# sunyinqi0508/AQuery2

Measured on AMD Instinct MI355X. Metric: rows/sec on h2o groupby 1e9-row, higher is better.
Workload: dtype int64

## Files before the change

### aquery2_amd/capi.py

```python
import ctypes as C
import os
import weakref

import numpy as np

HERE = os.path.dirname(os.path.abspath(__file__))

INT32, FLOAT, STR, DOUBLE, LDOUBLE, INT64, INT128, INT16, DATE, TIME, INT8 = range(11)
UINT32, UINT64, UINT128, UINT16, UINT8, BOOL = 11, 12, 13, 14, 15, 16
TIMESTAMP = 18
ERROR = 22
I128 = np.dtype([("lo", "<u8"), ("hi", "<i8")])
U128 = np.dtype([("lo", "<u8"), ("hi", "<u8")])
TAG2NP = {
    INT8: np.dtype(np.int8), INT16: np.dtype(np.int16), INT32: np.dtype(np.int32), INT64: np.dtype(np.int64),
    UINT8: np.dtype(np.uint8), UINT16: np.dtype(np.uint16), UINT32: np.dtype(np.uint32), UINT64: np.dtype(np.uint64),
    FLOAT: np.dtype(np.float32), DOUBLE: np.dtype(np.float64), BOOL: np.dtype(np.uint8), INT128: I128, UINT128: U128,
}
NP2TAG = {v: k for k, v in TAG2NP.items() if k != BOOL}
NP2TAG[np.dtype(np.bool_)] = BOOL
VEC_VEC, VEC_SCALAR, SCALAR_VEC = 0, 1, 2
LAYOUT_ROW, LAYOUT_FLAT = 0, 1
ORDER_ASC, ORDER_DESC, ORDER_NEG = 0, 1, 2
SEL_LOWER, SEL_UPPER = 0, 1
# ... 52 lines not shown
JOIN_INNER, JOIN_LEFT, JOIN_SEMI, JOIN_ANTI = range(4)
JOIN_ROUTE_PACKED, JOIN_ROUTE_WIDE, JOIN_ROUTE_LDS, JOIN_ROUTE_HBM = 1, 2, 4, 8
JOIN_KEYS_PROTOTYPES = {
    "aqg_join_keys_count": [C.c_void_p, C.c_int, C.c_int, C.c_void_p, C.c_void_p, C.c_uint32, C.c_void_p, C.c_uint32, C.POINTER(C.c_uint64)],
    "aqg_join_keys_pairs": [C.c_void_p, C.c_int, C.c_int, C.c_void_p, C.c_void_p, C.c_uint32, C.c_void_p, C.c_uint32, C.c_void_p, C.c_void_p,
                            C.c_uint64, C.POINTER(C.c_uint64)],
    "aqg_join_keys_lookup": [C.c_void_p, C.c_int, C.c_void_p, C.c_void_p, C.c_uint32, C.c_void_p, C.c_uint32, C.c_void_p],
    "aqg_join_last": [C.c_void_p, C.POINTER(C.c_uint32), C.POINTER(C.c_uint32), C.POINTER(C.c_uint32)],
    "aqg_join_tuple_slots": [C.c_int, C.c_void_p, C.c_void_p, C.c_uint32, C.c_uint32, C.c_void_p],
    "aqg_gather_fill": [C.c_void_p, C.c_int, C.c_void_p, C.c_void_p, C.c_uint32, C.c_void_p, C.c_void_p],
}
ASOF_BACKWARD, ASOF_FORWARD = 0, 1
ASOF_STRICT = 1
ASOF_ROUTE_LDS, ASOF_ROUTE_HBM, ASOF_ROUTE_NOKEYS, ASOF_ROUTE_PRESORTED = 1, 2, 4, 8
ASOF_PROTOTYPES = {
    "aqg_join_asof": [C.c_void_p, C.c_int, C.c_int, C.c_int, C.c_void_p, C.c_void_p, C.c_void_p, C.c_uint32, C.c_void_p, C.c_void_p, C.c_uint32,
                      C.c_int, C.c_void_p],
    "aqg_join_asof_last": [C.c_void_p, C.POINTER(C.c_uint32), C.POINTER(C.c_uint32), C.POINTER(C.c_uint32)],
}
STR_ROUTE_HOST, STR_ROUTE_DEVICE, STR_ROUTE_FALLBACK = 1, 2, 4
STR_PROTOTYPES = {
    "aqg_str_encode_last": [C.c_void_p, C.POINTER(C.c_uint32), C.POINTER(C.c_uint32)],
}
PLAN_FAST_LDS, PLAN_SMALL_LDS, PLAN_BIG_LDS, PLAN_DENSE, PLAN_PART_ONE, PLAN_PART_TWO, PLAN_PART_ROUND1, PLAN_PART_WIDE, PLAN_SORTED_TAIL, PLAN_HBM_TABLE, PLAN_BUILD_PARTITIONED, PLAN_GID_PARTITION, PLAN_PACKED_VALUES, PLAN_RANGE_PARTITIONS, PLAN_ROW_EMIT, PLAN_PACKED_KEYS, PLAN_BUILD_LOOKUP = (1 << i for i in range(17))


class AqgError(RuntimeError):
    def __init__(self, what, code, detail=""):
        super().__init__(f"{what}: status {code} {detail}")
        self.code = code


def lib_path():
    return os.path.join(HERE, "libaqg.so")


_LIB = None


def load_library():
    global _LIB
    if _LIB is None:
        p = lib_path()
        if not os.path.exists(p):
            raise FileNotFoundError(f"{p} not built: run `python -c 'import __graft_entry__ as g; g.build()'` "
                                    "or `make -C aquery2_amd/csrc`")
        lib = C.CDLL(p)
# ... 733 lines not shown

    def grouped_flatten(self, gb, x, keep=False):
        xd = self._dev(x)
        out = self.empty(xd.n, xd.dtype)
        self._chk(self.lib.aqg_grouped_flatten(self.ctx, gb.h, xd.tag, C.c_void_p(xd.ptr), C.c_void_p(out.ptr)), "aqg_grouped_flatten")
        return out if keep else out.to_host()

    def grouped_scan(self, gb, op, x, w=0, flat=False, keep=False, out=None):
        xd = self._dev(x)
        ot = self.lib.aqg_scan_out_dtype(op, xd.tag)
        out = out if out is not None else self.empty(xd.n, TAG2NP[ot])
        fn = self.lib.aqg_grouped_scan_flat if flat else self.lib.aqg_grouped_scan
        self._chk(fn(self.ctx, gb.h, op, xd.tag, C.c_void_p(xd.ptr), C.c_uint32(w), C.c_void_p(out.ptr)), "aqg_grouped_scan")
        return out if keep else out.to_host()

    def grouped_reduce_flat(self, gb, op, xflat):
        xd = self._dev(xflat)
        ot = self.lib.aqg_reduce_out_dtype(op, xd.tag)
        out = self.empty(gb.ngroups, TAG2NP[ot])
        self._chk(self.lib.aqg_grouped_reduce_flat(self.ctx, gb.h, op, xd.tag, C.c_void_p(xd.ptr), C.c_void_p(out.ptr)), "aqg_grouped_reduce_flat")
        self.sync()
        return out.to_host()

    def grouped_corr(self, gb, x, y):
        xd, yd = self._dev(x), self._dev(y)
        out = self.empty(gb.ngroups, np.float64)
        self._chk(self.lib.aqg_grouped_corr(self.ctx, gb.h, xd.tag, C.c_void_p(xd.ptr), yd.tag, C.c_void_p(yd.ptr), C.c_void_p(out.ptr)), "aqg_grouped_corr")
        self.sync()
        return out.to_host()

    def grouped_ewise(self, gb, op, v, s, kind=VEC_SCALAR, layout=LAYOUT_ROW, ot=None, keep=False, out=None):
        vd, sd = self._dev(v), self._dev(s)
        if ot is None:
            ot = self.lib.aqg_ewise_out_dtype(op, *((vd.tag, sd.tag) if kind == VEC_SCALAR else (sd.tag, vd.tag)))
        if ot == ERROR:
            raise AqgError("aqg_ewise_out_dtype", ERROR)
        out = out if out is not None else self.empty(vd.n, TAG2NP[ot])
        self._chk(self.lib.aqg_grouped_ewise(self.ctx, gb.h, layout, op, kind, vd.tag, C.c_void_p(vd.ptr), sd.tag, C.c_void_p(sd.ptr), ot,
                                             C.c_void_p(out.ptr)), "aqg_grouped_ewise")
        return out if keep else out.to_host()

    def join_pairs(self, build, probe):
        bd, pd = self._dev(build), self._dev(probe)
        m = C.c_uint64()
        self._chk(self.lib.aqg_join_count(self.ctx, bd.tag, C.c_void_p(bd.ptr), C.c_uint32(bd.n), C.c_void_p(pd.ptr),
                                          C.c_uint32(pd.n), C.byref(m)), "aqg_join_count")
# ... 87 lines not shown
```

### aquery2_amd/csrc/aqg_internal.hpp

```cpp
#pragma once
#include <hip/hip_runtime.h>

#include <cstdint>
#include <cstdio>
#include <cstring>
#include <string>
#include <unordered_map>
#include <vector>

#include "../../include/aqg.h"

struct aqg_pin { void* dptr; size_t bytes; std::vector<std::pair<void*, size_t>> regs; hipEvent_t ev; };

struct aqg_ctx {
    int device = 0;
    hipStream_t stream = nullptr;
    bool own_stream = false;
    int num_cu = 256;
    std::string err;
    char* ws = nullptr;
    size_t ws_cap = 0, ws_off = 0;
    hipEvent_t ev0 = nullptr, ev1 = nullptr;
    hipEvent_t evk0 = nullptr, evk1 = nullptr;
    hipEvent_t ev_flags = nullptr;
// ... 40 lines not shown
            (void)hipGetLastError();  \
            return AQG_ERR_HIP;                                                                \
        }                                                                                      \
    } while (0)

#define AQG_TRY(expr)                          \
    do {                                       \
        int _rc = (expr);                      \
        if (_rc != AQG_OK) return _rc;         \
    } while (0)

static inline int aqg_fail(aqg_ctx* ctx, int code, const char* msg) {
    if (ctx) ctx->err = msg;
    return code;
}
#define AQG_CHECK_ROWS(ctx, n, what) do { if ((uint64_t)(n) > (uint64_t)AQG_MAX_ROWS) return aqg_fail(ctx, AQG_ERR_ARG, what ": more than AQG_MAX_ROWS rows"); } while (0)
static inline uint32_t aqg_ceil_div(uint32_t n, uint32_t d) { return (uint32_t)(((uint64_t)n + d - 1) / d); }

struct aqg_switch_set {
    uint32_t p1_max, sorted_tail_min;
    int p1_bins;
    uint32_t select_small_max, select_split_min;
    double pw_sigma;
    bool disable_p1, disable_p1_cursors, disable_ranged, disable_pw_defer, disable_build_partition, debug_flags, str_host;
};
const aqg_switch_set& aqg_switches();

int aqg_ws_reset(aqg_ctx* ctx);
static inline void* aqg_pool_take(aqg_ctx* ctx, size_t need, size_t* cap) {
    if (ctx->pool_big && ctx->pool_big_cap >= need && ctx->pool_big_cap <= 2 * need) { void* p = ctx->pool_big; *cap = ctx->pool_big_cap; ctx->pool_big = nullptr; ctx->pool_big_cap = 0; return p; }
    int best = -1;
    const size_t slack = need * 4 > ((size_t)64 << 10) ? need * 4 : ((size_t)64 << 10);
    for (int i = 0; i < (int)ctx->pool.size(); ++i)
        if (ctx->pool[i].second >= need && ctx->pool[i].second <= slack && (best < 0 || ctx->pool[i].second < ctx->pool[best].second)) best = i;
    if (best < 0) return nullptr;
    void* p = ctx->pool[best].first;
    *cap = ctx->pool[best].second;
    ctx->pool_bytes -= *cap;
    ctx->pool[best] = ctx->pool.back();
    ctx->pool.pop_back();
    return p;
}
static inline void aqg_pool_give(aqg_ctx* ctx, void* p, size_t cap) {
    if (!p) return;
    if (ctx && cap && cap <= ((size_t)64 << 20) && ctx->pool.size() < 64 && ctx->pool_bytes + cap <= ((size_t)512 << 20)) { ctx->pool.emplace_back(p, cap); ctx->pool_bytes += cap; return; }
    if (ctx && cap > ((size_t)64 << 20) && cap <= ((size_t)8 << 30) && cap > ctx->pool_big_cap) {
        if (ctx->pool_big) (void)hipFree(ctx->pool_big);
// ... 17 lines not shown
    hipError_t e = hipSuccess;
    void* q = aqg_pool_alloc(ctx, need < 256 ? 256 : need, cap, &e);
    if (!q) { ctx->err = std::string("hipMalloc: ") + hipGetErrorString(e); return AQG_ERR_NOMEM; }
    *p = static_cast<T*>(q);
    return AQG_OK;
}
int aqg_ws_alloc(aqg_ctx* ctx, size_t bytes, void** out);
int aqg_ws_ensure(aqg_ctx* ctx, size_t bytes);
template <class T> static inline int aqg_ws_get(aqg_ctx* ctx, size_t count, T** out) {
    void* p = nullptr;
    int rc = aqg_ws_alloc(ctx, count * sizeof(T), &p);
    *out = static_cast<T*>(p);
    return rc;
}
int aqg_host_stage(aqg_ctx* ctx, size_t bytes, void** out);
int aqg_exclusive_scan_u32(aqg_ctx* ctx, uint32_t* d, uint64_t count, uint32_t* bsum);

struct aqg_groupby;
size_t aqg_postproc_ws_bytes(uint32_t n, uint32_t G, int esz);
int aqg_radix_by_group(aqg_ctx* ctx, aqg_groupby* g, uint32_t* row_ids_dev, const void* x, int esz, void* xout, bool ws_managed);
int aqg_group_offsets(aqg_ctx* ctx, const aqg_groupby* g, uint32_t* offsets_dev, uint32_t* bsum);
int aqg_flat_gid(aqg_ctx* ctx, aqg_groupby* g, const uint32_t** gid);
extern "C" int aqg_grouped_reduce_keyed(aqg_ctx* ctx, aqg_groupby* g, const uint32_t* gid_col, int op, int t, const void* x, void* out_dev);

struct aqg_comm;
int aqg_comm_allgather_internal(aqg_comm* c, const void* send_dev, void* recv_dev, size_t bytes);
aqg_ctx* aqg_comm_ctx(aqg_comm* c);
extern "C" int aqg_scan_minmax_seeded(aqg_ctx* ctx, int op, int t, const void* x, uint32_t n, const void* seed_host, void* out);

extern "C" int aqg_stats_dev(aqg_ctx* ctx, int t, const void* x, uint32_t n, int flags, void* out_dev48);
extern "C" int aqg_corr_sums_dev(aqg_ctx* ctx, int tx, const void* x, int ty, const void* y, uint32_t n, void* out_dev80);
int aqg_comm_scratch(aqg_comm* c, size_t send_bytes, size_t recv_bytes, void** send, void** recv);

constexpr int AQG_RED_SUMSQ = 64;

static inline void aqg_kernel_timer_begin(aqg_ctx* ctx) { if (!ctx->evk_frozen) (void)hipEventRecord(ctx->evk0, ctx->stream); }
static inline void aqg_kernel_timer_end(aqg_ctx* ctx) { if (!ctx->evk_frozen) { (void)hipEventRecord(ctx->evk1, ctx->stream); ctx->evk_valid = true; } }

static inline int aqg_check_launch(aqg_ctx* ctx, const char* what) {
    hipError_t e = hipGetLastError();
    if (e != hipSuccess) {
        ctx->err = std::string(what) + ": " + hipGetErrorString(e);
        return AQG_ERR_HIP;
    }
    return AQG_OK;
}
// ... 48 lines not shown
```

### aquery2_amd/csrc/ctx.hip

```cpp
#include <string_view>

#include <mutex>

#include "aqg_internal.hpp"

extern "C" {

const char* aqg_version(void) { return "aquery2_amd 0.1 (gfx950)"; }

size_t aqg_dtype_size(int dt) {
    switch (dt) {
    case AQG_INT8: case AQG_UINT8: case AQG_BOOL: case AQG_CHAR: return 1;
    case AQG_INT16: case AQG_UINT16: return 2;
    case AQG_INT32: case AQG_UINT32: case AQG_FLOAT: return 4;
    case AQG_INT64: case AQG_UINT64: case AQG_DOUBLE: return 8;
    case AQG_INT128: case AQG_UINT128: return 16;
    default: return 0;
    }
}
int aqg_long_type(int dt) {
    if (!aqg_dtype_size(dt)) return AQG_ERROR;
    if (dt_is_fp(dt)) return AQG_DOUBLE;
    return dt_is_unsigned(dt) ? AQG_UINT128 : AQG_INT128;
}
// ... 339 lines not shown
    AQG_HIP(ctx, hipEventElapsedTime(ms, ctx->ev0, ctx->ev1));
    return AQG_OK;
}

int aqg_last_kernel_ms(aqg_ctx* ctx, float* ms) {
    if (!ctx || !ms) return AQG_ERR_ARG;
    if (!ctx->evk_valid) return aqg_fail(ctx, AQG_ERR_ARG, "aqg_last_kernel_ms: no timed kernel yet");
    AQG_HIP(ctx, hipEventSynchronize(ctx->evk1));
    AQG_HIP(ctx, hipEventElapsedTime(ms, ctx->evk0, ctx->evk1));
    return AQG_OK;
}

}

const aqg_switch_set& aqg_switches() {
    auto num = [](const char* name, int dflt) { return getenv(name) ? atoi(getenv(name)) : dflt; };
    auto set = [](const char* name) { return getenv(name) != nullptr; };
    auto unum = [](const char* name, uint32_t dflt) { return getenv(name) ? (uint32_t)strtoul(getenv(name), nullptr, 10) : dflt; };
    static const aqg_switch_set s{
        .p1_max = (uint32_t)num("AQG_P1_MAX", 1024), .sorted_tail_min = (uint32_t)num("AQG_SORTED_TAIL_MIN", 1 << 24), .p1_bins = num("AQG_P1_BINS", 0),
        .select_small_max = unum("AQG_SELECT_SMALL_MAX", 256), .select_split_min = unum("AQG_SELECT_SPLIT_MIN", 1u << 20),
        .pw_sigma = getenv("AQG_PW_SIGMA") ? atof(getenv("AQG_PW_SIGMA")) : 6.0,
        .disable_p1 = set("AQG_DISABLE_P1"), .disable_p1_cursors = set("AQG_DISABLE_P1_CURSORS"), .disable_ranged = set("AQG_DISABLE_RANGED"),
        .disable_pw_defer = set("AQG_DISABLE_PW_DEFER"), .disable_build_partition = set("AQG_DISABLE_BUILD_PARTITION"),
        .debug_flags = set("AQG_DEBUG_FLAGS"), .str_host = set("AQG_STR_HOST")};
    return s;
}

int aqg_ws_reset(aqg_ctx* ctx) {
    ctx->ws_off = 0;
    return AQG_OK;
}
int aqg_ws_ensure(aqg_ctx* ctx, size_t bytes) {
    if (bytes <= ctx->ws_cap) return AQG_OK;
    AQG_HIP(ctx, hipSetDevice(ctx->device));
    AQG_HIP(ctx, hipStreamSynchronize(ctx->stream));
    size_t cap = ctx->ws_cap ? ctx->ws_cap : (size_t)1 << 20;
    while (cap < bytes) cap *= 2;
    if (bytes > ((size_t)4 << 30)) cap = (bytes + (((size_t)1 << 30) - 1)) & ~(((size_t)1 << 30) - 1);
    if (ctx->ws) { hipFree(ctx->ws); ctx->ws = nullptr; ctx->ws_cap = 0; }
    void* p = nullptr;
    hipError_t e = hipMalloc(&p, cap);
    if (e != hipSuccess) { ctx->err = std::string("workspace hipMalloc: ") + hipGetErrorString(e); (void)hipGetLastError(); return AQG_ERR_NOMEM; }
    ctx->ws = static_cast<char*>(p);
    ctx->ws_cap = cap;
    return AQG_OK;
}
// ... 21 lines not shown
```

### aquery2_amd/csrc/groupby.hip

```cpp
#include "groupby_plan.hpp"

size_t aqg_partition_ws_bytes(uint32_t n, int ksz, const AccSpec& as, uint32_t pbits);
int aqg_partition_aggregate(aqg_ctx* ctx, const KeySpec& ks, const AccSpec& as, uint32_t n, uint32_t pbits, uint32_t lcap, int need_count, GTable out, uint32_t out_cap);

int aqg_make_keyspec(aqg_ctx* ctx, int nkeys, const int* dts, const void* const* keys, uint32_t n, KeySpec* ks) {
    if (nkeys < 1 || nkeys > MAXKEYS) return aqg_fail(ctx, AQG_ERR_ARG, "group-by: 1..8 key columns");
    int bits = 0;
    ks->nkeys = nkeys;
    ks->range_known = 0; ks->range_lo = ks->range_hi = 0;
    for (int j = 0; j < nkeys; ++j) {
        if (!(dt_is_num(dts[j]) || dts[j] == AQG_BOOL)) return aqg_fail(ctx, AQG_ERR_DTYPE, "group-by: key dtype");
        if (dt_is_fp(dts[j])) return aqg_fail(ctx, AQG_ERR_DTYPE, "group-by: internal: floating key column reached the packed-key layer");
        if (!keys[j] && n) return aqg_fail(ctx, AQG_ERR_ARG, "group-by: null key column");
        ks->dt[j] = dts[j]; ks->col[j] = keys[j]; ks->shift[j] = bits;
        bits += 8 * (int)aqg_dtype_size(dts[j]);
    }
    ks->wide = bits > 64;
    if (ks->wide) for (int j = 0; j < nkeys; ++j) ks->shift[j] = 0;
    ks->total_bytes = bits / 8;
    return AQG_OK;
}

int aqg_add_acc(Plan* p, int kind, int dt, const void* col, int square, int part) {
    for (int a = 0; a < p->as.nacc; ++a)
// ... 383 lines not shown
    for (int attempt = 0; attempt < 12; ++attempt) {
        if (cur > n && n) cur = n;
        int rc = run_agg(ctx, ks, plan, n, (uint32_t)cur, for_build, h, gt_out, slot_gid_out, occ_out, dense_out);
        for (int again = 0; again < 3 && rc == AQG_ERR_RANGE_MISS; ++again) rc = run_agg(ctx, ks, plan, n, (uint32_t)cur, for_build, h, gt_out, slot_gid_out, occ_out, dense_out);
        if (rc != AQG_ERR_OVERFLOW) { if (rc == AQG_OK) h->hint_used = (uint32_t)cur; return rc; }
        if (n && cur >= n) return aqg_fail(ctx, AQG_ERR_OVERFLOW, "group-by: table overflow at full capacity");
        const uint64_t next = cur < (1ull << 25) && cur * 16 > (1ull << 25) ? (1ull << 25) : cur * 16;
        cur = plan.sj && cur < 3072 && next > 3072 ? 3072 : next;
    }
    return aqg_fail(ctx, AQG_ERR_OVERFLOW, "group-by: table overflow");
}

extern "C" {

void aqg_groupby_destroy(aqg_groupby* g) {
    if (!g) return;
    aqg_ctx* ctx = g->ctx;
    for (int k = 0; k < MAXKEYS; ++k) aqg_pool_give(ctx, g->keys_out[k], g->cap_keys[k]);
    for (int j = 0; j < MAXAGG; ++j) aqg_pool_give(ctx, g->results[j], g->cap_results[j]);
    aqg_pool_give(ctx, g->first_rows, g->cap_first);
    aqg_pool_give(ctx, g->counts, g->cap_counts);
    aqg_pool_give(ctx, g->reversemap, g->cap_rows * 4);
    if (g->scratch) aqg_groupby_destroy(g->scratch);
    if (g->scratch2) aqg_groupby_destroy(g->scratch2);
    if (g->scratch3) aqg_groupby_destroy(g->scratch3);
    aqg_pool_give(ctx, g->flat_off, g->cap_flat_off);
    aqg_pool_give(ctx, g->flat_heads, g->cap_flat_heads);
    aqg_pool_give(ctx, g->flat_short, g->cap_flat_short);
    aqg_pool_give(ctx, g->flat_gid, g->cap_flat_gid);
    if (g->first_rows64) hipFree(g->first_rows64);
    for (int i = 0; i < 2 * MAXKEYS; ++i) if (g->norm_buf[i]) hipFree(g->norm_buf[i]);
    if (g->xkeys) hipFree(g->xkeys);
    if (g->xvals) hipFree(g->xvals);
    delete g;
}
uint32_t aqg_groupby_ngroups(const aqg_groupby* g) { return g ? g->ngroups : 0; }
uint32_t aqg_groupby_nrows(const aqg_groupby* g) { return g ? g->n : 0; }
const uint32_t* aqg_groupby_reversemap(const aqg_groupby* g) { return g && g->has_reversemap ? g->reversemap : nullptr; }
const uint32_t* aqg_groupby_counts(const aqg_groupby* g) { return g && g->has_counts ? g->counts : nullptr; }
const uint32_t* aqg_groupby_first_rows(const aqg_groupby* g) { return g && !g->sharded ? g->first_rows : nullptr; }
uint32_t aqg_groupby_plan(const aqg_groupby* g) { return g ? g->plan_bits : 0; }
const void* aqg_groupby_agg_result(const aqg_groupby* g, int j) { return g && j >= 0 && j < g->nagg ? g->results[j] : nullptr; }

int aqg_groupby_agg(aqg_ctx* ctx, int nkeys, const int* key_dtypes, const void* const* keys, int naggs, const int* ops,
                    const int* val_dtypes, const void* const* vals, uint32_t n, uint32_t max_groups_hint, aqg_groupby** out) {
    if (!ctx || !out || !key_dtypes || !keys) return aqg_fail(ctx, AQG_ERR_ARG, "aqg_groupby_agg: bad argument");
    AQG_CHECK_ROWS(ctx, n, "aqg_groupby_agg");
// ... 50 lines not shown
```

### aquery2_amd/csrc/groupby_handle.hpp

```cpp
#pragma once
#include <cstddef>
#include <cstdint>

struct aqg_ctx;
constexpr int MAXKEYS = 8, MAXACC = 8, MAXAGG = 8;

struct aqg_groupby {
    aqg_ctx* ctx = nullptr;
    uint32_t n = 0, ngroups = 0;
    int nkeys = 0;
    int key_dt[MAXKEYS] = {0};
    int key_esz[MAXKEYS] = {0};
    bool has_counts = false, has_reversemap = false;
    void* keys_out[MAXKEYS] = {nullptr};
    uint32_t* first_rows = nullptr;
    uint32_t* counts = nullptr;
    uint32_t* reversemap = nullptr;
    void* results[MAXAGG] = {nullptr};
    int nagg = 0;
    int res_dt[MAXAGG] = {0};
    size_t cap_keys[MAXKEYS] = {0}, cap_first = 0, cap_counts = 0, cap_rows = 0, cap_results[MAXAGG] = {0};
    uint32_t hint_used = 0;
    uint32_t plan_bits = 0;
    int64_t* first_rows64 = nullptr;
    size_t cap_first64 = 0;
    bool sharded = false;
    int nuser = 0;
    int user_dt[MAXKEYS] = {0};
    const void* user_col[MAXKEYS] = {nullptr};
    int user_norm[MAXKEYS] = {0};
    void* norm_buf[2 * MAXKEYS] = {nullptr};
    size_t cap_norm[2 * MAXKEYS] = {0};
    bool build_assigned = false;
    bool no_lookup_build = false;
    bool no_sorted_tail = false;
    bool no_pack = false;
    bool no_wide_part = false;
    uint32_t wide_rows = 0;
    uint32_t wide_seed = 0;
    bool dense_exact = false;
    bool range_valid = false; int range_nkeys = 0; uint32_t range_n = 0;
    const void* range_col[MAXKEYS] = {}; int range_dt[MAXKEYS] = {}; long long range_min[MAXKEYS] = {}, range_max[MAXKEYS] = {};
    aqg_groupby* scratch = nullptr;
    aqg_groupby* scratch2 = nullptr;
    aqg_groupby* scratch3 = nullptr;
    uint32_t* flat_off = nullptr; uint32_t* flat_heads = nullptr; uint32_t* flat_short = nullptr; uint32_t* flat_gid = nullptr;
    size_t cap_flat_off = 0, cap_flat_heads = 0, cap_flat_short = 0, cap_flat_gid = 0;
    bool flat_valid = false, flat_gid_valid = false;
    uint32_t flat_short_w = 0;
    void* xkeys = nullptr; void* xvals = nullptr;
    size_t cap_xkeys = 0, cap_xvals = 0;
};
```

### aquery2_amd/csrc/grouped_reduce.hip

```cpp
#include "groupby_plan.hpp"

namespace {
int dense_id_keys(aqg_ctx* ctx, aqg_groupby* g, const uint32_t* gid_col, KeySpec* ks, aqg_groupby** h) {
    const int kdt = AQG_UINT32;
    const void* kcol = gid_col;
    AQG_TRY(aqg_make_keyspec(ctx, 1, &kdt, &kcol, g->n, ks));
    ks->range_known = 1; ks->range_lo = 0; ks->range_hi = (long long)g->ngroups - 1;
    if (!g->scratch) g->scratch = new aqg_groupby();
    *h = g->scratch;
    (*h)->ctx = ctx; (*h)->n = g->n; (*h)->has_reversemap = false;
    return AQG_OK;
}
}

extern "C" {

namespace {
__global__ void __launch_bounds__(256) corr_final_kernel(const aqg_i128* __restrict__ sx, const aqg_i128* __restrict__ sx2, const aqg_i128* __restrict__ sy,
                                                        const aqg_i128* __restrict__ sy2, const aqg_i128* __restrict__ sxy, const uint32_t* __restrict__ counts,
                                                        uint32_t G, double* __restrict__ out) {
    for (uint32_t g = blockIdx.x * blockDim.x + threadIdx.x; g < G; g += gridDim.x * blockDim.x) {
        const aqg_i128 len = i128_from_u64(counts[g]);
        const double a = i128_to_double(i128_mul(len, sxy[g])) - i128_to_double(i128_mul(sx[g], sy[g]));
        const double b = i128_to_double(i128_mul(len, sx2[g])) - i128_to_double(i128_mul(sx[g], sx[g]));
// ... 35 lines not shown
    if (!dt_is_num(t)) return aqg_fail(ctx, AQG_ERR_DTYPE, "aqg_grouped_reduce: value dtype");
    const uint32_t G = g->ngroups, n = g->n;
    if (G == 0) return AQG_OK;
    if (op == AQG_RED_LAST) return aqg_gather(ctx, t, x, g->first_rows, G, out_dev);
    KeySpec ks;
    aqg_groupby* h = nullptr;
    AQG_TRY(dense_id_keys(ctx, g, g->reversemap, &ks, &h));
    if (op == AQG_RED_FIRST) {
        Plan plan;
        memset(&plan, 0, sizeof plan);
        plan.nagg = 1;
        plan.agg[0].op = AQG_RED_MAX; plan.agg[0].dt = AQG_UINT64; plan.agg[0].acc1 = plan.agg[0].acc2 = plan.agg[0].acc3 = -1;
        plan.agg[0].acc0 = aqg_add_acc(&plan, ACC_MAX, AQG_NONE, nullptr, 0);
        AQG_TRY(aqg_run_with_retry(ctx, ks, plan, n, G, false, h, nullptr, nullptr));
        uint32_t* rows = nullptr;
        AQG_TRY(aqg_ws_reset(ctx));
        AQG_TRY(aqg_ws_get(ctx, G, &rows));
        hipLaunchKernelGGL(take_rows_kernel, dim3(aqg_grid(ctx, G, 256, 1, 8)), dim3(256), 0, ctx->stream, (const uint64_t*)h->results[0], G, rows);
        return aqg_gather(ctx, t, x, rows, G, out_dev);
    }
    return aqg_grouped_reduce_keyed(ctx, g, g->reversemap, op, t, x, out_dev);
}

int aqg_grouped_corr(aqg_ctx* ctx, aqg_groupby* g, int tx, const void* x, int ty, const void* y, double* out_dev) {
    if (!ctx || !g || ((!x || !y) && g->n) || !out_dev) return aqg_fail(ctx, AQG_ERR_ARG, "aqg_grouped_corr: bad argument");
    if (!g->has_reversemap || !g->has_counts) return aqg_fail(ctx, AQG_ERR_ARG, "aqg_grouped_corr: handle has no reversemap (use aqg_groupby_build)");
    auto small_int = [](int dt) { return dt == AQG_INT8 || dt == AQG_INT16 || dt == AQG_INT32 || dt == AQG_UINT8 || dt == AQG_UINT16 || dt == AQG_UINT32; };
    if (!small_int(tx) || !small_int(ty)) return aqg_fail(ctx, AQG_ERR_DTYPE, "aqg_grouped_corr: integer columns of up to four bytes (others: aqg_corr per group)");
    const uint32_t G = g->ngroups, n = g->n;
    if (G == 0) return AQG_OK;
    const int pt = (tx == AQG_UINT32 || ty == AQG_UINT32) ? AQG_UINT32 : AQG_INT32;
    size_t cap = 0;
    void* xy = aqg_pool_alloc(ctx, (size_t)n * 4 + 64, &cap);
    if (!xy) return aqg_fail(ctx, AQG_ERR_NOMEM, "aqg_grouped_corr: product column");
    int rc = aqg_ewise(ctx, AQG_OP_MUL, AQG_VEC_VEC, tx, x, ty, y, pt, xy, n);
    if (rc == AQG_OK) {
        KeySpec ks;
        aqg_groupby* h = nullptr;
        rc = dense_id_keys(ctx, g, g->reversemap, &ks, &h);
        size_t sums_cap = 0;
        void* sums = aqg_pool_alloc(ctx, (size_t)G * 80 + 64, &sums_cap);
        if (!sums) rc = aqg_fail(ctx, AQG_ERR_NOMEM, "aqg_grouped_corr: sums");
        const int ops5[5] = {AQG_RED_SUM, AQG_RED_SUMSQ, AQG_RED_SUM, AQG_RED_SUMSQ, AQG_RED_SUM};
        const int dts5[5] = {tx, tx, ty, ty, pt};
        const void* vals5[5] = {x, x, y, y, xy};
        auto slot = [&](int j) { return static_cast<char*>(sums) + (size_t)j * G * 16; };
        auto pass = [&](int first, int count) -> int {
            Plan plan;
            AQG_TRY(aqg_make_plan(ctx, count, ops5 + first, dts5 + first, vals5 + first, n, &plan));
            AQG_TRY(aqg_run_with_retry(ctx, ks, plan, n, G, false, h, nullptr, nullptr));
            if (h->ngroups != G) return aqg_fail(ctx, AQG_ERR_ARG, "aqg_grouped_corr: group ids are not dense");
            for (int j = 0; j < count; ++j) AQG_HIP(ctx, hipMemcpyAsync(slot(first + j), h->results[j], (size_t)G * 16, hipMemcpyDeviceToDevice, ctx->stream));
            return AQG_OK;
        };
        if (rc == AQG_OK) {
            if (G <= 3072) { rc = pass(0, 4); if (rc == AQG_OK) rc = pass(4, 1); }
            else for (int j = 0; j < 5 && rc == AQG_OK; ++j) rc = pass(j, 1);
        }
        if (rc == AQG_OK) {
            hipLaunchKernelGGL(corr_final_kernel, dim3(aqg_grid(ctx, G, 256, 1, 8)), dim3(256), 0, ctx->stream, (const aqg_i128*)slot(0), (const aqg_i128*)slot(1),
                               (const aqg_i128*)slot(2), (const aqg_i128*)slot(3), (const aqg_i128*)slot(4), g->counts, G, out_dev);
            rc = aqg_check_launch(ctx, "corr_final_kernel");
        }
        if (sums) aqg_pool_give(ctx, sums, sums_cap);
    }
    aqg_pool_give(ctx, xy, cap);
    return rc;
}

}
```

### include/aqg.h

```cpp
#ifndef AQG_H
#define AQG_H

#include <stddef.h>
#include <stdint.h>

#ifdef __cplusplus
extern "C" {
#endif

typedef enum aqg_dtype {
    AQG_INT32 = 0, AQG_FLOAT = 1, AQG_STR = 2, AQG_DOUBLE = 3, AQG_LDOUBLE = 4,
    AQG_INT64 = 5, AQG_INT128 = 6, AQG_INT16 = 7, AQG_DATE = 8, AQG_TIME = 9,
    AQG_INT8 = 10, AQG_UINT32 = 11, AQG_UINT64 = 12, AQG_UINT128 = 13,
    AQG_UINT16 = 14, AQG_UINT8 = 15, AQG_BOOL = 16, AQG_VECTOR = 17,
    AQG_TIMESTAMP = 18, AQG_CHAR = 19, AQG_SV = 20, AQG_NONE = 21, AQG_ERROR = 22
} aqg_dtype;

enum {
    AQG_OK = 0,
    AQG_ERR_HIP = 1,
    AQG_ERR_DTYPE = 2,
    AQG_ERR_ARG = 3,
    AQG_ERR_NOMEM = 4,
    AQG_ERR_NODEVICE = 5,
// ... 140 lines not shown

int aqg_grouped_reduce(aqg_ctx* ctx, const aqg_groupby* g, int op, int t, const void* x, void* out_dev);

const uint32_t* aqg_groupby_offsets(aqg_groupby* g);
int aqg_grouped_flatten(aqg_ctx* ctx, aqg_groupby* g, int t, const void* x, void* out_flat);
int aqg_grouped_scan_flat(aqg_ctx* ctx, aqg_groupby* g, int op, int t, const void* xflat, uint32_t w, void* out_flat);
int aqg_grouped_scan(aqg_ctx* ctx, aqg_groupby* g, int op, int t, const void* x, uint32_t w, void* out_flat);
int aqg_grouped_reduce_flat(aqg_ctx* ctx, aqg_groupby* g, int op, int t, const void* xflat, void* out_dev);
int aqg_grouped_corr(aqg_ctx* ctx, aqg_groupby* g, int tx, const void* x, int ty, const void* y, double* out_dev);
enum { AQG_LAYOUT_ROW = 0, AQG_LAYOUT_FLAT = 1 };
int aqg_grouped_ewise(aqg_ctx* ctx, aqg_groupby* g, int layout, int op, int kind,
                      int vt, const void* v, int st, const void* s_dev, int ot, void* out);

int aqg_groupby_agg(aqg_ctx* ctx, int nkeys, const int* key_dtypes, const void* const* keys,
                    int naggs, const int* ops, const int* val_dtypes, const void* const* vals,
                    uint32_t n, uint32_t max_groups_hint, aqg_groupby** out);
const void* aqg_groupby_agg_result(const aqg_groupby* g, int j);
enum { AQG_PLAN_FAST_LDS = 1, AQG_PLAN_SMALL_LDS = 2, AQG_PLAN_BIG_LDS = 4, AQG_PLAN_DENSE = 8, AQG_PLAN_PART_ONE = 16, AQG_PLAN_PART_TWO = 32,
       AQG_PLAN_PART_ROUND1 = 64, AQG_PLAN_PART_WIDE = 128, AQG_PLAN_SORTED_TAIL = 256, AQG_PLAN_HBM_TABLE = 512, AQG_PLAN_BUILD_PARTITIONED = 1024, AQG_PLAN_GID_PARTITION = 2048 ,
       AQG_PLAN_PACKED_VALUES = 4096 ,
       AQG_PLAN_RANGE_PARTITIONS = 8192 ,
       AQG_PLAN_ROW_EMIT = 16384 ,
       AQG_PLAN_PACKED_KEYS = 32768 ,
       AQG_PLAN_BUILD_LOOKUP = 65536  };
uint32_t aqg_groupby_plan(const aqg_groupby* g);

int aqg_join_count(aqg_ctx* ctx, int t, const void* build_keys, uint32_t nb,
                   const void* probe_keys, uint32_t np, uint64_t* m_host);
int aqg_join_pairs(aqg_ctx* ctx, int t, const void* build_keys, uint32_t nb,
                   const void* probe_keys, uint32_t np,
                   uint32_t* probe_rows_out, uint32_t* build_rows_out, uint64_t capacity, uint64_t* m_host);
int aqg_join_lookup(aqg_ctx* ctx, int t, const void* build_keys, uint32_t nb,
                    const void* probe_keys, uint32_t np, uint32_t* build_row_of_probe);

enum { AQG_JOIN_INNER = 0, AQG_JOIN_LEFT = 1, AQG_JOIN_SEMI = 2, AQG_JOIN_ANTI = 3 };
int aqg_join_keys_count(aqg_ctx* ctx, int kind, int nkeys, const int* key_dtypes,
                        const void* const* build_keys, uint32_t nb,
                        const void* const* probe_keys, uint32_t np, uint64_t* m_host);
int aqg_join_keys_pairs(aqg_ctx* ctx, int kind, int nkeys, const int* key_dtypes,
                        const void* const* build_keys, uint32_t nb,
                        const void* const* probe_keys, uint32_t np,
                        uint32_t* probe_rows_out, uint32_t* build_rows_out, uint64_t capacity, uint64_t* m_host);
int aqg_join_keys_lookup(aqg_ctx* ctx, int nkeys, const int* key_dtypes,
                         const void* const* build_keys, uint32_t nb,
                         const void* const* probe_keys, uint32_t np, uint32_t* build_row_of_probe);
enum { AQG_JOIN_ROUTE_PACKED = 1, AQG_JOIN_ROUTE_WIDE = 2, AQG_JOIN_ROUTE_LDS = 4, AQG_JOIN_ROUTE_HBM = 8 };
int aqg_join_last(aqg_ctx* ctx, uint32_t* routes, uint32_t* build_groups, uint32_t* table_slots);
int aqg_join_tuple_slots(int nkeys, const int* key_dtypes, const void* const* host_keys, uint32_t n, uint32_t table_slots,
// ... 57 lines not shown
```

Before: 811.2 billion.

## Add direct LDS-atomic grouped correlation kernel computing all five sums in one pass

Adds a route for grouped_corr on small integer columns. One kernel reads the group ids and x/y once and accumulates sum x, x², y, y² and xy per group in LDS with 64-bit atomics, then widens to 128-bit. It replaces the older path that built an xy product column, derived dense keys and ran several grouped-reduce passes. In exchange it adds a host sync to check a flag that catches non-dense group ids, and it depends on the group count fitting in LDS.

Result: slower. 793.8 billion (-2.1%).

```diff
diff --git a/aquery2_amd/capi.py b/aquery2_amd/capi.py
--- a/aquery2_amd/capi.py
+++ b/aquery2_amd/capi.py
@@ -98,7 +98,7 @@
 STR_PROTOTYPES = {
     "aqg_str_encode_last": [C.c_void_p, C.POINTER(C.c_uint32), C.POINTER(C.c_uint32)],
 }
-PLAN_FAST_LDS, PLAN_SMALL_LDS, PLAN_BIG_LDS, PLAN_DENSE, PLAN_PART_ONE, PLAN_PART_TWO, PLAN_PART_ROUND1, PLAN_PART_WIDE, PLAN_SORTED_TAIL, PLAN_HBM_TABLE, PLAN_BUILD_PARTITIONED, PLAN_GID_PARTITION, PLAN_PACKED_VALUES, PLAN_RANGE_PARTITIONS, PLAN_ROW_EMIT, PLAN_PACKED_KEYS, PLAN_BUILD_LOOKUP = (1 << i for i in range(17))
+PLAN_FAST_LDS, PLAN_SMALL_LDS, PLAN_BIG_LDS, PLAN_DENSE, PLAN_PART_ONE, PLAN_PART_TWO, PLAN_PART_ROUND1, PLAN_PART_WIDE, PLAN_SORTED_TAIL, PLAN_HBM_TABLE, PLAN_BUILD_PARTITIONED, PLAN_GID_PARTITION, PLAN_PACKED_VALUES, PLAN_RANGE_PARTITIONS, PLAN_ROW_EMIT, PLAN_PACKED_KEYS, PLAN_BUILD_LOOKUP, PLAN_GROUPED_DIRECT = (1 << i for i in range(18))
 
 
 class AqgError(RuntimeError):
@@ -878,6 +878,9 @@
         self.sync()
         return out.to_host()
 
+    def grouped_corr_passes(self, ngroups):
+        return self.lib.aqg_grouped_corr_passes(C.c_uint32(ngroups))
+
     def grouped_corr(self, gb, x, y):
         xd, yd = self._dev(x), self._dev(y)
         out = self.empty(gb.ngroups, np.float64)
diff --git a/aquery2_amd/csrc/aqg_internal.hpp b/aquery2_amd/csrc/aqg_internal.hpp
--- a/aquery2_amd/csrc/aqg_internal.hpp
+++ b/aquery2_amd/csrc/aqg_internal.hpp
@@ -86,7 +86,7 @@
     int p1_bins;
     uint32_t select_small_max, select_split_min;
     double pw_sigma;
-    bool disable_p1, disable_p1_cursors, disable_ranged, disable_pw_defer, disable_build_partition, debug_flags, str_host;
+    bool disable_p1, disable_p1_cursors, disable_ranged, disable_pw_defer, disable_build_partition, disable_corr_direct, debug_flags, str_host;
 };
 const aqg_switch_set& aqg_switches();
 
@@ -150,6 +150,10 @@
 int aqg_group_offsets(aqg_ctx* ctx, const aqg_groupby* g, uint32_t* offsets_dev, uint32_t* bsum);
 int aqg_flat_gid(aqg_ctx* ctx, aqg_groupby* g, const uint32_t** gid);
 extern "C" int aqg_grouped_reduce_keyed(aqg_ctx* ctx, aqg_groupby* g, const uint32_t* gid_col, int op, int t, const void* x, void* out_dev);
+struct aqg_i128;
+int aqg_corr_direct_plan(uint32_t G, int masks[5]);
+bool aqg_corr_direct_applies(const aqg_groupby* g, int tx, const void* x, int ty, const void* y);
+int aqg_corr_direct_sums(aqg_ctx* ctx, const aqg_groupby* g, int tx, const void* x, int ty, const void* y, aqg_i128* sums128, void* scratch);
 
 struct aqg_comm;
 int aqg_comm_allgather_internal(aqg_comm* c, const void* send_dev, void* recv_dev, size_t bytes);
diff --git a/aquery2_amd/csrc/ctx.hip b/aquery2_amd/csrc/ctx.hip
--- a/aquery2_amd/csrc/ctx.hip
+++ b/aquery2_amd/csrc/ctx.hip
@@ -385,7 +385,7 @@
         .select_small_max = unum("AQG_SELECT_SMALL_MAX", 256), .select_split_min = unum("AQG_SELECT_SPLIT_MIN", 1u << 20),
         .pw_sigma = getenv("AQG_PW_SIGMA") ? atof(getenv("AQG_PW_SIGMA")) : 6.0,
         .disable_p1 = set("AQG_DISABLE_P1"), .disable_p1_cursors = set("AQG_DISABLE_P1_CURSORS"), .disable_ranged = set("AQG_DISABLE_RANGED"),
-        .disable_pw_defer = set("AQG_DISABLE_PW_DEFER"), .disable_build_partition = set("AQG_DISABLE_BUILD_PARTITION"),
+        .disable_pw_defer = set("AQG_DISABLE_PW_DEFER"), .disable_build_partition = set("AQG_DISABLE_BUILD_PARTITION"), .disable_corr_direct = set("AQG_DISABLE_CORR_DIRECT"),
         .debug_flags = set("AQG_DEBUG_FLAGS"), .str_host = set("AQG_STR_HOST")};
     return s;
 }
diff --git a/aquery2_amd/csrc/groupby.hip b/aquery2_amd/csrc/groupby.hip
--- a/aquery2_amd/csrc/groupby.hip
+++ b/aquery2_amd/csrc/groupby.hip
@@ -429,7 +429,6 @@
     aqg_pool_give(ctx, g->counts, g->cap_counts);
     aqg_pool_give(ctx, g->reversemap, g->cap_rows * 4);
     if (g->scratch) aqg_groupby_destroy(g->scratch);
-    if (g->scratch2) aqg_groupby_destroy(g->scratch2);
     if (g->scratch3) aqg_groupby_destroy(g->scratch3);
     aqg_pool_give(ctx, g->flat_off, g->cap_flat_off);
     aqg_pool_give(ctx, g->flat_heads, g->cap_flat_heads);
diff --git a/aquery2_amd/csrc/groupby_handle.hpp b/aquery2_amd/csrc/groupby_handle.hpp
--- a/aquery2_amd/csrc/groupby_handle.hpp
+++ b/aquery2_amd/csrc/groupby_handle.hpp
@@ -42,7 +42,6 @@
     bool range_valid = false; int range_nkeys = 0; uint32_t range_n = 0;
     const void* range_col[MAXKEYS] = {}; int range_dt[MAXKEYS] = {}; long long range_min[MAXKEYS] = {}, range_max[MAXKEYS] = {};
     aqg_groupby* scratch = nullptr;
-    aqg_groupby* scratch2 = nullptr;
     aqg_groupby* scratch3 = nullptr;
     uint32_t* flat_off = nullptr; uint32_t* flat_heads = nullptr; uint32_t* flat_short = nullptr; uint32_t* flat_gid = nullptr;
     size_t cap_flat_off = 0, cap_flat_heads = 0, cap_flat_short = 0, cap_flat_gid = 0;
diff --git a/aquery2_amd/csrc/grouped_corr_direct.hip b/aquery2_amd/csrc/grouped_corr_direct.hip
--- /dev/null
+++ b/aquery2_amd/csrc/grouped_corr_direct.hip
@@ -0,0 +1,180 @@
+#include "aqg_internal.hpp"
+#include "dev_common.hpp"
+#include "groupby_handle.hpp"
+
+namespace {
+enum : int { SX = 1, SX2 = 2, SY = 4, SY2 = 8, SXY = 16 };
+enum : uint32_t { SG_X = 1, SG_Y = 2, SG_XX = 4, SG_YY = 8, SG_XY = 16 };
+constexpr size_t CORR_LDS_MAX = 160 * 1024;
+constexpr int CR = 8;
+
+template <int W> struct uint_of;
+template <> struct uint_of<1> { using type = uint8_t; };
+template <> struct uint_of<2> { using type = uint16_t; };
+template <> struct uint_of<4> { using type = uint32_t; };
+
+template <int W> __device__ inline uint32_t promote32(typename uint_of<W>::type raw, bool sgn) {
+    if constexpr (W == 1) return sgn ? (uint32_t)(int32_t)(int8_t)raw : (uint32_t)raw;
+    else if constexpr (W == 2) return sgn ? (uint32_t)(int32_t)(int16_t)raw : (uint32_t)raw;
+    else return raw;
+}
+__device__ inline unsigned long long ext64(uint32_t v, bool sgn) { return sgn ? (unsigned long long)(long long)(int32_t)v : (unsigned long long)v; }
+
+template <int W> __device__ inline void load_step(const void* col, size_t base, uint32_t T, uint32_t tid, typename uint_of<W>::type (&o)[CR]) {
+    using U = typename uint_of<W>::type;
+    const U* p = static_cast<const U*>(col) + base + 4 * (size_t)tid;
+    const pack<U, 4> a = *reinterpret_cast<const pack<U, 4>*>(p), b = *reinterpret_cast<const pack<U, 4>*>(p + 4 * (size_t)T);
+#pragma unroll
+    for (int r = 0; r < 4; ++r) { o[r] = a.v[r]; o[4 + r] = b.v[r]; }
+}
+
+template <int WX, int WY, int MASK>
+__global__ void __launch_bounds__(1024) corr_direct_kernel(const uint32_t* __restrict__ ids, const void* __restrict__ x, const void* __restrict__ y, uint32_t n, uint32_t G,
+                                                           uint32_t sg, unsigned long long* __restrict__ sums , uint32_t* __restrict__ flag) {
+    constexpr bool NX = (MASK & (SX | SX2 | SXY)) != 0, NY = (MASK & (SY | SY2 | SXY)) != 0;
+    constexpr int NK = __builtin_popcount(MASK);
+    using UX = typename uint_of<WX>::type;
+    using UY = typename uint_of<WY>::type;
+    extern __shared__ __align__(16) unsigned char smem_raw[];
+    unsigned long long* acc = reinterpret_cast<unsigned long long*>(smem_raw);
+    const uint32_t T = blockDim.x, tid = threadIdx.x;
+    for (uint32_t i = tid; i < NK * G; i += T) acc[i] = 0;
+    __syncthreads();
+    auto slot = [&](int bit) { return acc + (size_t)__builtin_popcount(MASK & (bit - 1)) * G; };
+    auto add = [&](unsigned long long* p, unsigned long long v) { (void)__hip_atomic_fetch_add(p, v, __ATOMIC_RELAXED, __HIP_MEMORY_SCOPE_WORKGROUP); };
+    bool bad = false;
+    auto row = [&](uint32_t gid, UX xr, UY yr) {
+        if (gid >= G) { bad = true; return; }
+        const uint32_t xv = NX ? promote32<WX>(xr, sg & SG_X) : 0, yv = NY ? promote32<WY>(yr, sg & SG_Y) : 0;
+        if constexpr (MASK & SX) add(slot(SX) + gid, ext64(xv, sg & SG_X));
+        if constexpr (MASK & SX2) add(slot(SX2) + gid, ext64(xv * xv, sg & SG_XX));
+        if constexpr (MASK & SY) add(slot(SY) + gid, ext64(yv, sg & SG_Y));
+        if constexpr (MASK & SY2) add(slot(SY2) + gid, ext64(yv * yv, sg & SG_YY));
+        if constexpr (MASK & SXY) add(slot(SXY) + gid, ext64(xv * yv, sg & SG_XY));
+    };
+    struct Step { uint32_t id[CR]; UX x[CR]; UY y[CR]; };
+    auto load = [&](size_t base, Step& s) {
+        load_step<4>(ids, base, T, tid, s.id);
+        if constexpr (NX) load_step<WX>(x, base, T, tid, s.x);
+        if constexpr (NY) load_step<WY>(y, base, T, tid, s.y);
+    };
+    const size_t step = (size_t)CR * T;
+    const uint64_t nfull = n / step, stride = gridDim.x;
+    uint64_t t = blockIdx.x;
+    Step cur = {};
+    if (t < nfull) load(t * step, cur);
+    while (t < nfull) {
+        const uint64_t tn = t + stride;
+        Step nxt = {};
+        load((tn < nfull ? tn : t) * step, nxt);
+        __builtin_amdgcn_sched_barrier(0);
+#pragma unroll
+        for (int r = 0; r < CR; ++r) row(cur.id[r], cur.x[r], cur.y[r]);
+        cur = nxt;
+        t = tn;
+    }
+    if (blockIdx.x == 0)
+        for (size_t i = nfull * step + tid; i < n; i += T) {
+            UX xr = 0; UY yr = 0;
+            if constexpr (NX) xr = static_cast<const UX*>(x)[i];
+            if constexpr (NY) yr = static_cast<const UY*>(y)[i];
+            row(ids[i], xr, yr);
+        }
+    __syncthreads();
+    int k = 0;
+#pragma unroll
+    for (int s = 0; s < 5; ++s) {
+        if (!(MASK & (1 << s))) continue;
+        for (uint32_t g = tid; g < G; g += T) {
+            const unsigned long long v = acc[(size_t)k * G + g];
+            if (v) (void)__hip_atomic_fetch_add(sums + (size_t)s * G + g, v, __ATOMIC_RELAXED, __HIP_MEMORY_SCOPE_AGENT);
+        }
+        ++k;
+    }
+    if (bad) (void)__hip_atomic_fetch_or(flag, 1u, __ATOMIC_RELAXED, __HIP_MEMORY_SCOPE_AGENT);
+}
+
+__global__ void __launch_bounds__(256) corr_widen_kernel(const unsigned long long* __restrict__ sums, uint32_t G, uint32_t sg, aqg_i128* __restrict__ out) {
+    for (uint32_t i = blockIdx.x * blockDim.x + threadIdx.x; i < 5 * G; i += gridDim.x * blockDim.x) {
+        const uint32_t s = i / G;
+        out[i] = (sg >> s) & 1 ? i128_from_i64((long long)sums[i]) : i128_from_u64(sums[i]);
+    }
+}
+
+bool small_int(int dt) { return dt == AQG_INT8 || dt == AQG_INT16 || dt == AQG_INT32 || dt == AQG_UINT8 || dt == AQG_UINT16 || dt == AQG_UINT32; }
+
+uint32_t corr_direct_sign(int tx, int ty) {
+    return (dt_is_unsigned(tx) ? 0 : SG_X) | (dt_is_unsigned(ty) ? 0 : SG_Y) | (tx == AQG_UINT32 ? 0 : SG_XX) | (ty == AQG_UINT32 ? 0 : SG_YY) |
+           (tx == AQG_UINT32 || ty == AQG_UINT32 ? 0 : SG_XY);
+}
+
+using corr_kernel_t = void (*)(const uint32_t*, const void*, const void*, uint32_t, uint32_t, uint32_t, unsigned long long*, uint32_t*);
+template <int WX, int WY> corr_kernel_t corr_kernel_of_mask(int mask) {
+    switch (mask) {
+    case SX | SX2 | SY | SY2 | SXY: return corr_direct_kernel<WX, WY, (SX | SX2 | SY | SY2 | SXY)>;
+    case SX | SX2 | SXY: return corr_direct_kernel<WX, WY, (SX | SX2 | SXY)>;
+    case SXY: return corr_direct_kernel<WX, WY, SXY>;
+    case SX | SX2: return corr_direct_kernel<WX, 4, (SX | SX2)>;
+    case SX: return corr_direct_kernel<WX, 4, SX>;
+    case SX2: return corr_direct_kernel<WX, 4, SX2>;
+    case SY | SY2: return corr_direct_kernel<4, WY, (SY | SY2)>;
+    case SY: return corr_direct_kernel<4, WY, SY>;
+    case SY2: return corr_direct_kernel<4, WY, SY2>;
+    }
+    return nullptr;
+}
+template <int WX> corr_kernel_t corr_kernel_of_y(int wy, int mask) {
+    return wy == 1 ? corr_kernel_of_mask<WX, 1>(mask) : wy == 2 ? corr_kernel_of_mask<WX, 2>(mask) : corr_kernel_of_mask<WX, 4>(mask);
+}
+corr_kernel_t corr_kernel_of(int wx, int wy, int mask) {
+    return wx == 1 ? corr_kernel_of_y<1>(wy, mask) : wx == 2 ? corr_kernel_of_y<2>(wy, mask) : corr_kernel_of_y<4>(wy, mask);
+}
+}
+
+int aqg_corr_direct_plan(uint32_t G, int masks[5]) {
+    if (G == 0) return 0;
+    const size_t K = CORR_LDS_MAX / (8 * (size_t)G);
+    int np = 0;
+    if (K >= 5) masks[np++] = SX | SX2 | SY | SY2 | SXY;
+    else if (K >= 3) { masks[np++] = SX | SX2 | SXY; masks[np++] = SY | SY2; }
+    else if (K == 2) { masks[np++] = SX | SX2; masks[np++] = SY | SY2; masks[np++] = SXY; }
+    else if (K == 1) for (int s = 0; s < 5; ++s) masks[np++] = 1 << s;
+    return np;
+}
+
+extern "C" int aqg_grouped_corr_passes(uint32_t ngroups) {
+    int masks[5];
+    return aqg_corr_direct_plan(ngroups, masks);
+}
+
+bool aqg_corr_direct_applies(const aqg_groupby* g, int tx, const void* x, int ty, const void* y) {
+    if (aqg_switches().disable_corr_direct || !small_int(tx) || !small_int(ty) || !aqg_grouped_corr_passes(g->ngroups)) return false;
+    return (((uintptr_t)g->reversemap | (uintptr_t)x | (uintptr_t)y) & 15) == 0;
+}
+
+int aqg_corr_direct_sums(aqg_ctx* ctx, const aqg_groupby* g, int tx, const void* x, int ty, const void* y, aqg_i128* sums128, void* scratch) {
+    const uint32_t G = g->ngroups, n = g->n;
+    int masks[5];
+    const int np = aqg_corr_direct_plan(G, masks);
+    if (!np) return aqg_fail(ctx, AQG_ERR_ARG, "aqg_grouped_corr: too many groups for the direct route");
+    unsigned long long* sums = static_cast<unsigned long long*>(scratch);
+    uint32_t* flag = reinterpret_cast<uint32_t*>(sums + (size_t)5 * G);
+    AQG_HIP(ctx, hipMemsetAsync(scratch, 0, (size_t)G * 40 + 4, ctx->stream));
+    const uint32_t sg = corr_direct_sign(tx, ty);
+    aqg_kernel_timer_begin(ctx);
+    for (int p = 0; p < np; ++p) {
+        const size_t lds = (size_t)__builtin_popcount(masks[p]) * G * 8;
+        const uint32_t block = 1024;
+        const uint64_t steps = n / ((uint64_t)CR * block), cap = (uint64_t)ctx->num_cu;
+        const uint32_t grid = (uint32_t)(steps < 1 ? 1 : steps < cap ? steps : cap);
+        const corr_kernel_t kern = corr_kernel_of((int)aqg_dtype_size(tx), (int)aqg_dtype_size(ty), masks[p]);
+        if (!kern) return aqg_fail(ctx, AQG_ERR_ARG, "aqg_grouped_corr: no kernel for this pass");
+        AQG_TRY(aqg_allow_lds(ctx, reinterpret_cast<const void*>(kern), lds));
+        hipLaunchKernelGGL(kern, dim3(grid), dim3(block), lds, ctx->stream, g->reversemap, x, y, n, G, sg, sums, flag);
+        AQG_TRY(aqg_check_launch(ctx, "corr_direct_kernel"));
+    }
+    aqg_kernel_timer_end(ctx);
+    const uint32_t sg5 = (sg & SG_X ? 1u : 0u) | (sg & SG_XX ? 2u : 0u) | (sg & SG_Y ? 4u : 0u) | (sg & SG_YY ? 8u : 0u) | (sg & SG_XY ? 16u : 0u);
+    hipLaunchKernelGGL(corr_widen_kernel, dim3(aqg_grid(ctx, (uint64_t)5 * G, 256, 1, 8)), dim3(256), 0, ctx->stream, sums, G, sg5, sums128);
+    return aqg_check_launch(ctx, "corr_widen_kernel");
+}
diff --git a/aquery2_amd/csrc/grouped_reduce.hip b/aquery2_amd/csrc/grouped_reduce.hip
--- a/aquery2_amd/csrc/grouped_reduce.hip
+++ b/aquery2_amd/csrc/grouped_reduce.hip
@@ -81,13 +81,9 @@
     return aqg_grouped_reduce_keyed(ctx, g, g->reversemap, op, t, x, out_dev);
 }
 
-int aqg_grouped_corr(aqg_ctx* ctx, aqg_groupby* g, int tx, const void* x, int ty, const void* y, double* out_dev) {
-    if (!ctx || !g || ((!x || !y) && g->n) || !out_dev) return aqg_fail(ctx, AQG_ERR_ARG, "aqg_grouped_corr: bad argument");
-    if (!g->has_reversemap || !g->has_counts) return aqg_fail(ctx, AQG_ERR_ARG, "aqg_grouped_corr: handle has no reversemap (use aqg_groupby_build)");
-    auto small_int = [](int dt) { return dt == AQG_INT8 || dt == AQG_INT16 || dt == AQG_INT32 || dt == AQG_UINT8 || dt == AQG_UINT16 || dt == AQG_UINT32; };
-    if (!small_int(tx) || !small_int(ty)) return aqg_fail(ctx, AQG_ERR_DTYPE, "aqg_grouped_corr: integer columns of up to four bytes (others: aqg_corr per group)");
+namespace {
+int corr_by_plans(aqg_ctx* ctx, aqg_groupby* g, int tx, const void* x, int ty, const void* y, void* sums) {
     const uint32_t G = g->ngroups, n = g->n;
-    if (G == 0) return AQG_OK;
     const int pt = (tx == AQG_UINT32 || ty == AQG_UINT32) ? AQG_UINT32 : AQG_INT32;
     size_t cap = 0;
     void* xy = aqg_pool_alloc(ctx, (size_t)n * 4 + 64, &cap);
@@ -97,9 +93,6 @@
         KeySpec ks;
         aqg_groupby* h = nullptr;
         rc = dense_id_keys(ctx, g, g->reversemap, &ks, &h);
-        size_t sums_cap = 0;
-        void* sums = aqg_pool_alloc(ctx, (size_t)G * 80 + 64, &sums_cap);
-        if (!sums) rc = aqg_fail(ctx, AQG_ERR_NOMEM, "aqg_grouped_corr: sums");
         const int ops5[5] = {AQG_RED_SUM, AQG_RED_SUMSQ, AQG_RED_SUM, AQG_RED_SUMSQ, AQG_RED_SUM};
         const int dts5[5] = {tx, tx, ty, ty, pt};
         const void* vals5[5] = {x, x, y, y, xy};
@@ -116,15 +109,44 @@
             if (G <= 3072) { rc = pass(0, 4); if (rc == AQG_OK) rc = pass(4, 1); }
             else for (int j = 0; j < 5 && rc == AQG_OK; ++j) rc = pass(j, 1);
         }
-        if (rc == AQG_OK) {
-            hipLaunchKernelGGL(corr_final_kernel, dim3(aqg_grid(ctx, G, 256, 1, 8)), dim3(256), 0, ctx->stream, (const aqg_i128*)slot(0), (const aqg_i128*)slot(1),
-                               (const aqg_i128*)slot(2), (const aqg_i128*)slot(3), (const aqg_i128*)slot(4), g->counts, G, out_dev);
-            rc = aqg_check_launch(ctx, "corr_final_kernel");
-        }
-        if (sums) aqg_pool_give(ctx, sums, sums_cap);
+        if (rc == AQG_OK) g->plan_bits = h->plan_bits;
     }
     aqg_pool_give(ctx, xy, cap);
     return rc;
 }
+}
+
+int aqg_grouped_corr(aqg_ctx* ctx, aqg_groupby* g, int tx, const void* x, int ty, const void* y, double* out_dev) {
+    if (!ctx || !g || ((!x || !y) && g->n) || !out_dev) return aqg_fail(ctx, AQG_ERR_ARG, "aqg_grouped_corr: bad argument");
+    if (!g->has_reversemap || !g->has_counts) return aqg_fail(ctx, AQG_ERR_ARG, "aqg_grouped_corr: handle has no reversemap (use aqg_groupby_build)");
+    auto small_int = [](int dt) { return dt == AQG_INT8 || dt == AQG_INT16 || dt == AQG_INT32 || dt == AQG_UINT8 || dt == AQG_UINT16 || dt == AQG_UINT32; };
+    if (!small_int(tx) || !small_int(ty)) return aqg_fail(ctx, AQG_ERR_DTYPE, "aqg_grouped_corr: integer columns of up to four bytes (others: aqg_corr per group)");
+    const uint32_t G = g->ngroups;
+    if (G == 0) return AQG_OK;
+    const bool direct = aqg_corr_direct_applies(g, tx, x, ty, y);
+    size_t sums_cap = 0;
+    char* sums = static_cast<char*>(aqg_pool_alloc(ctx, (size_t)G * 120 + 64, &sums_cap));
+    if (!sums) return aqg_fail(ctx, AQG_ERR_NOMEM, "aqg_grouped_corr: sums");
+    uint32_t* flag = reinterpret_cast<uint32_t*>(sums + (size_t)G * 120);
+    int rc = direct ? aqg_corr_direct_sums(ctx, g, tx, x, ty, y, reinterpret_cast<aqg_i128*>(sums), sums + (size_t)G * 80) : corr_by_plans(ctx, g, tx, x, ty, y, sums);
+    if (rc == AQG_OK) {
+        auto slot = [&](int j) { return reinterpret_cast<const aqg_i128*>(sums + (size_t)j * G * 16); };
+        hipLaunchKernelGGL(corr_final_kernel, dim3(aqg_grid(ctx, G, 256, 1, 8)), dim3(256), 0, ctx->stream, slot(0), slot(1), slot(2), slot(3), slot(4), g->counts, G, out_dev);
+        rc = aqg_check_launch(ctx, "corr_final_kernel");
+    }
+    if (rc == AQG_OK && direct) {
+        void* st = nullptr;
+        rc = aqg_host_stage(ctx, 16, &st);
+        if (rc == AQG_OK) {
+            hipError_t e = hipMemcpyAsync(st, flag, 4, hipMemcpyDeviceToHost, ctx->stream);
+            if (e == hipSuccess) e = hipStreamSynchronize(ctx->stream);
+            if (e != hipSuccess) { ctx->err = std::string("aqg_grouped_corr: flag: ") + hipGetErrorString(e); (void)hipGetLastError(); rc = AQG_ERR_HIP; }
+            else if (*static_cast<const uint32_t*>(st)) rc = aqg_fail(ctx, AQG_ERR_ARG, "aqg_grouped_corr: group ids are not dense");
+            else g->plan_bits = AQG_PLAN_GROUPED_DIRECT;
+        }
+    }
+    aqg_pool_give(ctx, sums, sums_cap);
+    return rc;
+}
 
 }
diff --git a/include/aqg.h b/include/aqg.h
--- a/include/aqg.h
+++ b/include/aqg.h
@@ -186,8 +186,10 @@
        AQG_PLAN_RANGE_PARTITIONS = 8192 ,
        AQG_PLAN_ROW_EMIT = 16384 ,
        AQG_PLAN_PACKED_KEYS = 32768 ,
-       AQG_PLAN_BUILD_LOOKUP = 65536  };
+       AQG_PLAN_BUILD_LOOKUP = 65536 ,
+       AQG_PLAN_GROUPED_DIRECT = 131072  };
 uint32_t aqg_groupby_plan(const aqg_groupby* g);
+int aqg_grouped_corr_passes(uint32_t ngroups);
 
 int aqg_join_count(aqg_ctx* ctx, int t, const void* build_keys, uint32_t nb,
                    const void* probe_keys, uint32_t np, uint64_t* m_host);
```
